# peterropac/Aegolius

Measured on AMD Instinct MI355X. Metric: Mpoints/sec SDF eval, 1024^3 grid, 10-prim smooth-union tree, higher is better.
Workload: dtype f32

## Files before the change

aegolius_amd/_engine.py:

```python
import atexit
import contextlib
import ctypes
import importlib.util
import os
import sys
import threading

import numpy as np

_HERE = os.path.dirname(os.path.abspath(__file__))
LIB_PATH = os.path.join(_HERE, "libsdfk.so")

MODE_AUTO, MODE_INTERPRET, MODE_SPECIALIZED, MODE_NOCULL = 0, 1, 2, 3
(FLAVOUR_PLAIN_ARRAY, FLAVOUR_PLAIN_GRID, FLAVOUR_TILE_ARRAY, FLAVOUR_TILE_GRID, FLAVOUR_TILE_MASK, FLAVOUR_ROWS_ARRAY,
 FLAVOUR_ROWS_GRID, FLAVOUR_ROWS_MASK, FLAVOUR_ROWS2D_ARRAY, FLAVOUR_ROWS2D_GRID, FLAVOUR_RAYS, FLAVOUR_OCCUPANCY) = range(12)
FLAVOUR_FLAGS = 0x100
FLAVOUR_XY = 0x200

_c = ctypes
_vp, _i64, _int, _sz = _c.c_void_p, _c.c_int64, _c.c_int, _c.c_size_t
_fp = _c.POINTER(_c.c_float)

SIGNATURES = {
    "sdfk_abi_version": (_int, []),
    "sdfk_device_count": (_int, []),
    "sdfk_last_error": (_c.c_char_p, []),
    "sdfk_program_create": (_vp, [_vp, _sz, _vp, _sz, _vp, _sz, _int]),
    "sdfk_program_destroy": (None, [_vp]),
    "sdfk_program_set_params": (_int, [_vp, _vp, _sz]),
    "sdfk_program_set_cull": (_int, [_vp, _vp, _sz, _vp]),
    "sdfk_program_source": (_c.c_char_p, [_vp]),
    "sdfk_program_compile_check": (_int, [_vp, _c.POINTER(_sz)]),
    "sdfk_program_chain_members": (_int, [_vp]),
    "sdfk_program_compile_flavour": (_int, [_vp, _int, _c.POINTER(_sz), _c.POINTER(_c.c_double)]),
    "sdfk_debug_compile_external": (_int, [_vp, _int, _c.POINTER(_sz)]),
    "sdfk_debug_jit_stats": (None, [_c.POINTER(_i64), _c.POINTER(_c.c_double)]),
    "sdfk_jit_drain": (None, []),
    "sdfk_jit_cancel": (None, []),
    "sdfk_debug_set_rtc_defs": (None, [_c.c_char_p]),
    "sdfk_eval_device": (_int, [_vp, _vp, _i64, _i64, _vp, _vp, _int]),
    "sdfk_eval_device_rows": (_int, [_vp, _vp, _i64, _i64, _i64, _vp, _vp, _int]),
    "sdfk_eval_device_rows2d": (_int, [_vp, _vp, _i64, _i64, _i64, _vp, _vp, _int]),
    "sdfk_eval_device_rows2d_xy": (_int, [_vp, _vp, _i64, _i64, _i64, _vp, _vp, _int]),
    "sdfk_debug_cells_stats": (None, [_int, _c.POINTER(_c.c_longlong)]),
    "sdfk_debug_rays_stats": (None, [_int, _c.POINTER(_c.c_longlong)]),
    "sdfk_eval_device_rows3d": (_int, [_vp, _vp, _i64, _i64, _i64, _i64, _i64, _vp, _vp, _int]),
    "sdfk_debug_row_masks": (_int, [_vp, _vp, _i64, _i64, _i64, _vp, _c.POINTER(_i64), _c.POINTER(_int), _vp]),
    "sdfk_eval_grid_sharded": (_int, [_vp, _vp, _i64, _vp, _i64, _vp, _i64, _int, _vp, _vp, _int]),
    "sdfk_eval_grid_sharded_device": (_int, [_vp, _vp, _i64, _vp, _i64, _vp, _i64, _int, _vp, _int, _vp, _int]),
    "sdfk_eval_device_aux": (_int, [_vp, _vp, _i64, _i64, _vp, _int, _i64, _vp, _vp, _int]),
    "sdfk_eval_grid_aux": (_int, [_vp, _vp, _i64, _vp, _i64, _vp, _i64, _i64, _i64, _vp, _int, _i64, _vp, _vp, _int]),
    "sdfk_field_min": (_int, [_vp, _i64, _c.POINTER(_c.c_float), _vp]),
    "sdfk_grid_box_average": (_int, [_vp, _i64, _i64, _i64, _int, _int, _int, _int, _vp, _vp]),
    "sdfk_grid_edge_detect": (_int, [_vp, _i64, _i64, _i64, _vp, _vp]),
    "sdfk_debug_box_variant": (_int, [_i64, _i64, _i64, _int, _int, _int, _c.POINTER(_int)]),
    "sdfk_grid_signed": (_int, [_vp, _i64, _i64, _i64, _c.c_float, _int, _vp, _vp]),
    "sdfk_grid_boundary_mask": (_int, [_vp, _i64, _c.c_float, _vp, _vp]),
    "sdfk_grid_signed_slab": (_int, [_vp, _i64, _i64, _vp, _i64, _i64, _i64, _int, _vp, _vp]),
    "sdfk_eval_host": (_int, [_vp, _vp, _int, _i64, _i64, _vp, _int, _int]),
# ... 141 lines not shown


def check(rc, what):
    if rc != 0:
        raise SdfkError("%s failed (%d): %s" % (what, rc, last_error()))


def device_count():
    return lib().sdfk_device_count()


def require_gpu():
    if device_count() < 1:
        raise SdfkError("aegolius_amd: no HIP device visible - SDF evaluation runs on an MI355X only "
                        "(there is no CPU path)")


def jit_stats():
    n, t = _i64(0), _c.c_double(0.0)
    lib().sdfk_debug_jit_stats(ctypes.byref(n), ctypes.byref(t))
    return n.value, t.value


def _ptr(a):
    return a.ctypes.data_as(_vp) if a is not None and a.size else None


def _release(owner, attr, destroy):
    try:
        h = getattr(owner, attr, None)
        setattr(owner, attr, None)
        if h and _lib is not None:
            getattr(_lib, destroy)(_vp(h))
    except Exception:
        pass


def coords_n(shape):
    if len(shape) != 2 or shape[0] != 3:
        raise ValueError("coordinates must have shape (3, N); got %r" % (tuple(shape),))
    return int(shape[1])


def host_coords(co, dtype=None):
    co = np.asarray(co)
    coords_n(co.shape)
# ... 543 lines not shown
```

aegolius_amd/csrc/sdfk.hip:

```cpp
#include <hip/hip_runtime.h>
#include <hip/hiprtc.h>

#include <chrono>
#include <algorithm>
#include <atomic>
#include <cmath>
#include <condition_variable>
#include <cstdio>
#include <cstdlib>
#include <cstring>
#include <deque>
#include <functional>
#include <map>
#include <memory>
#include <mutex>
#include <thread>
#include <string>
#include <vector>
#include <dirent.h>
#include <dlfcn.h>
#include <fcntl.h>
#include <signal.h>
#include <spawn.h>
#include <sys/wait.h>
// ... 989 lines not shown
        std::lock_guard<std::mutex> lk(mu);
        jobs.clear();
        cv.notify_all();
    }
    ~BuildWorker() {
        {
            std::lock_guard<std::mutex> lk(mu);
            stop = true;
            cv.notify_all();
        }
        for (std::thread& t : threads)
            if (t.joinable()) t.join();
    }
};
static BuildWorker g_builds;
extern "C" void sdfk_jit_drain(void) { g_builds.drain(); }
extern "C" void sdfk_jit_cancel(void) {
    g_cancel_builds.store(true);
    g_builds.drop_queued();
    g_builds.drain();
}
static std::atomic<long long> g_compile_count{0};
static std::atomic<long long> g_compile_micros{0};
extern "C" void sdfk_debug_jit_stats(int64_t* builds, double* seconds) {
    if (builds) *builds = g_compile_count.load();
    if (seconds) *seconds = (double)g_compile_micros.load() * 1e-6;
}

static std::shared_ptr<CodeObject> code_entry(const std::string& key) {
    std::lock_guard<std::mutex> lk(g_code_mu);
    std::shared_ptr<CodeObject>& e = g_code[key];
    if (!e) e = std::make_shared<CodeObject>();
    return e;
}
static void code_build(const std::shared_ptr<CodeObject>& e, const std::string& src, int rwb, bool external = false) {
    const auto t0 = std::chrono::steady_clock::now();
    std::vector<char> co;
    std::string log;
    bool from_disk = false;
    std::string disk_path;
    const int rc = rtc_compile(src, &co, &log, rwb, &from_disk, &disk_path, external);
    const double dt = std::chrono::duration<double>(std::chrono::steady_clock::now() - t0).count();
    if (!from_disk) {
        g_compile_count++;
        g_compile_micros += (long long)(dt * 1e6);
    }
// ... 10 lines not shown
    }
    e->cv.notify_all();
}
template <typename MakeSource>
static std::shared_ptr<CodeObject> code_get(const std::string& key, MakeSource make_source, int rwb, bool wait) {
    std::shared_ptr<CodeObject> e = code_entry(key);
    std::unique_lock<std::mutex> lk(e->mu);
    if (e->state == 3 && std::chrono::steady_clock::now() - e->failed_at > std::chrono::seconds(30)) e->state = 0;
    if (e->state == 0) {
        e->state = 1;
        lk.unlock();
        const std::string src = make_source();
        if (wait || !rtc_helper_available()) {
            code_build(e, src, rwb);
        } else {
            g_builds.post([e, src, rwb] { code_build(e, src, rwb, true); });
        }
        return e;
    }
    if (wait) e->cv.wait(lk, [&] { return e->state != 1; });
    return e;
}
static std::string flavour_key(const sdfk_program* p, int flavour, int rwb, int with_flags = 0) {
    return p->key + "|f" + std::to_string(flavour) + ((with_flags & 1) ? "s" : "") + ((with_flags & 2) ? "x" : "") + "|" + rtc_option_key(rwb);
}
static std::string flavour_source(const sdfk_program* p, int flavour, int with_flags = 0) {
    return std::string((with_flags & 1) ? "#define SDFK_FLAGS 1\n" : "") + ((with_flags & 2) ? "#define SDFK_XY 1\n" : "") +
           sdfk_generate_source(g_ops, SDFK_OP_COUNT, p->code.data(), p->code.size() / 2, p->result_reg, p->sites, flavour,
                                &p->sites_all);
}

extern "C" int sdfk_program_chain_members(const sdfk_program* p) {
    return p && p->chain_mode ? p->chain_members : 0;
}
extern "C" int sdfk_program_compile_check(sdfk_program* p, size_t* code_size) {
    if (!p) return fail(-1, "null program");
    size_t total = 0;
    const int rwb = rows_geo(p);
    for (int f = 0; f < SDFK_FL_COUNT; ++f) {
        if (f == SDFK_FL_RAYS) continue;
        if (f == SDFK_FL_OCCUPANCY) continue;
        if (p->sites.empty() && f != SDFK_FL_PLAIN_ARRAY && f != SDFK_FL_PLAIN_GRID) continue;
        if (p->chain_mode && (f == SDFK_FL_TILE_ARRAY || f == SDFK_FL_TILE_GRID || f == SDFK_FL_TILE_MASK || f == SDFK_FL_ROWS_MASK)) continue;
        std::shared_ptr<CodeObject> e = code_get(flavour_key(p, f, rwb), [&] { return flavour_source(p, f); }, rwb, true);
        if (e->state != 2) return fail(-3, e->error);
        total += e->co.size();
    }
    if (code_size) *code_size = total;
    return 0;
}
extern "C" int sdfk_program_compile_flavour(sdfk_program* p, int flavour, size_t* code_size, double* seconds) {
    if (!p) return fail(-1, "null program");
    int with_flags = 0;
    if (flavour >= 0 && (flavour & SDFK_FLAVOUR_FLAGS)) with_flags |= 1;
    if (flavour >= 0 && (flavour & SDFK_FLAVOUR_XY)) with_flags |= 2;
    if (flavour >= 0) flavour &= ~(SDFK_FLAVOUR_FLAGS | SDFK_FLAVOUR_XY);
    if (flavour < 0 || flavour >= SDFK_FL_COUNT) return fail(-1, "sdfk_program_compile_flavour: unknown flavour");
    if (p->sites.empty() && flavour != SDFK_FL_PLAIN_ARRAY && flavour != SDFK_FL_PLAIN_GRID && flavour != SDFK_FL_RAYS &&
        flavour != SDFK_FL_OCCUPANCY)
        return fail(-2, "sdfk_program_compile_flavour: the program has no cull sites");
    if (with_flags && flavour == SDFK_FL_RAYS)
        return fail(-2, "sdfk_program_compile_flavour: the ray flavour has no flag-writing or two-row build");
    if (with_flags && flavour == SDFK_FL_OCCUPANCY)
        return fail(-2, "sdfk_program_compile_flavour: the occupancy flavour has no flag-writing or two-row build");
    if ((with_flags & 2) && flavour != SDFK_FL_PLAIN_ARRAY && flavour != SDFK_FL_ROWS2D_ARRAY)
        return fail(-2, "sdfk_program_compile_flavour: two-row coordinates exist for the plain and the flat row-block array kernels");
    if ((with_flags & 1) && (flavour == SDFK_FL_TILE_ARRAY || flavour == SDFK_FL_TILE_GRID || flavour == SDFK_FL_TILE_MASK ||
                       flavour == SDFK_FL_ROWS_MASK))
        return fail(-2, "sdfk_program_compile_flavour: this flavour has no flag-writing build");
    const int rwb = rows_geo(p);
    const auto t0 = std::chrono::steady_clock::now();
    std::shared_ptr<CodeObject> e =
        code_get(flavour_key(p, flavour, rwb, with_flags), [&] { return flavour_source(p, flavour, with_flags); }, rwb, true);
    if (e->state != 2) return fail(-3, e->error);
    if (code_size) *code_size = e->co.size();
    if (seconds) *seconds = std::chrono::duration<double>(std::chrono::steady_clock::now() - t0).count();
    return 0;
}

extern "C" int sdfk_debug_compile_external(sdfk_program* p, int flavour, size_t* code_size) {
    if (!p) return fail(-1, "null program");
    if (flavour < 0 || flavour >= SDFK_FL_COUNT) return fail(-1, "sdfk_debug_compile_external: unknown flavour");
    if (p->sites.empty() && flavour != SDFK_FL_PLAIN_ARRAY && flavour != SDFK_FL_PLAIN_GRID && flavour != SDFK_FL_RAYS &&
// ... 261 lines not shown
        for (const uint2& x : sp) {
            if (x.y == 0xffffffffu) ++all;
            else { sum += x.y; mx = std::max<unsigned long long>(mx, x.y); if (x.y == 0) ++empty; }
        }
        {
            std::lock_guard<std::mutex> lk(g_cells_stats_mu);
            g_cells_stats[0] = (long long)nf; g_cells_stats[1] = (long long)nc; g_cells_stats[2] = (long long)head;
            g_cells_stats[3] = (long long)cap; g_cells_stats[4] = (long long)sum; g_cells_stats[5] = (long long)mx;
            g_cells_stats[6] = (long long)all; g_cells_stats[7] = (long long)empty;
        }
        if (trace) fprintf(stderr, "[sdfk cells] %d members: fine %ux%ux%u = %llu cells (2^%u planes x 2^%u blocks x 2^%u windows), coarse %llu; pool %u of %llu entries; "
                "fine lists: mean %.1f max %llu, %llu without a list, %llu empty\n", p->chain_members, fine.ncx, fine.ncy, fine.ncz, nf, fine.lx, fine.ly, fine.lz, nc,
                head, cap, (double)sum / (double)std::max<unsigned long long>(1, nf - all - empty), mx, all, empty);
    }
    out->lv = fine;
    out->sph = b + o_fsph;
    out->span = b + o_fspan;
    out->cand = b + o_pool;
    out->enabled = 1u;
    out->ncells = (unsigned)nf;
    return 0;
}

static int run(sdfk_program* p, const SrcArray* arr, const SrcGrid* grid, long long n, float* d_out, void* stream_,
               int mode, bool vec_ok, long long row_len = 0, const float* aux = nullptr, long long aux_stride = 0,
               bool flat = false, long long plane_rows = 0, long long plane_phase = 0, unsigned* d_flags = nullptr,
               unsigned thr_key = 0, bool xy = false) {
    if (!p) return fail(-1, "null program");
    if (n < 0) return fail(-1, "negative point count");
    if (p->n_aux > 0 && (!aux || aux_stride < n))
        return fail(-1, "this program reads auxiliary fields (staged evaluation): use sdfk_eval_device_aux / sdfk_eval_grid_aux");
    if (n == 0) return 0;
    if (mode == SDFK_MODE_AUTO) mode = g_default_mode;
    if (d_flags && (mode == SDFK_MODE_AUTO || mode == SDFK_MODE_INTERPRET)) mode = SDFK_MODE_SPECIALIZED;
    if (xy) {
        if (!arr || p->n_aux > 0) return fail(-1, "two-row coordinates: array source, no auxiliary fields");
        if (mode == SDFK_MODE_AUTO || mode == SDFK_MODE_INTERPRET) mode = SDFK_MODE_SPECIALIZED;
    }
    hipStream_t stream = (hipStream_t)stream_;
    int device = 0;
    HIPCHK(hipGetDevice(&device));
    DevState* d = nullptr;
    int rc = ensure_resident(p, device, stream, &d);
    if (rc) return rc;

    long long n4 = vec_ok ? (n / 4) * 4 : 0;
    long long tail = n - n4;

    static const long long spec_limit = [] {
        const char* e = getenv("SDFK_SPECIALIZE_LIMIT");
// ... 7 lines not shown
    }();
    if (mode == SDFK_MODE_AUTO && (long long)(p->code.size() / 2) > spec_limit && p->interp_ok && !p->chain_mode && !d_flags)
        mode = SDFK_MODE_INTERPRET;

    RowGeom rg;
    int flavour = arr ? SDFK_FL_PLAIN_ARRAY : SDFK_FL_PLAIN_GRID;
    const long long grow = grid ? (grid->n2 > 1 ? (long long)grid->n2 : (long long)grid->n1) : 0;
    if (!p->sites.empty() && mode != SDFK_MODE_NOCULL && mode != SDFK_MODE_INTERPRET) {
        if (arr && rows_geometry(n, row_len, &rg, (flat || d_flags) ? 0 : plane_rows, plane_phase, p->chain_mode))
            flavour = (flat || xy) ? SDFK_FL_ROWS2D_ARRAY : SDFK_FL_ROWS_ARRAY;
        else if (arr && vec_ok && !p->chain_mode && !d_flags && !xy) flavour = SDFK_FL_TILE_ARRAY;
        else if (grid && grid->start % grow == 0 &&
                 rows_geometry(n, grow, &rg, (grid->n2 > 1 && !d_flags) ? (long long)grid->n1 : 0,
                               grid->n2 > 1 ? (grid->start / grow) % (long long)grid->n1 : 0, p->chain_mode))
            flavour = grid->n2 > 1 ? SDFK_FL_ROWS_GRID : SDFK_FL_ROWS2D_GRID;
        else if (grid && vec_ok && !p->chain_mode && !d_flags) flavour = SDFK_FL_TILE_GRID;
        if (!p->chain_mode && (long long)(p->code.size() / 2) > rows_limit &&
            (flavour == SDFK_FL_ROWS_ARRAY || flavour == SDFK_FL_ROWS2D_ARRAY || flavour == SDFK_FL_ROWS_GRID || flavour == SDFK_FL_ROWS2D_GRID)) {
            const bool is_arr = arr != nullptr;
            if (vec_ok && !d_flags && !xy) flavour = is_arr ? SDFK_FL_TILE_ARRAY : SDFK_FL_TILE_GRID;
            else if (!d_flags) flavour = is_arr ? SDFK_FL_PLAIN_ARRAY : SDFK_FL_PLAIN_GRID;
        }
    }
    std::shared_ptr<SpecModule> sk;
    if (mode != SDFK_MODE_INTERPRET) {
        static const bool async_jit = [] { const char* e = getenv("SDFK_ASYNC_JIT"); return !(e && e[0] == '0'); }();
        const bool wait = mode != SDFK_MODE_AUTO || !p->interp_ok || !async_jit;
        std::string err;
        sk = get_module(p, device, flavour, wait, &err, (d_flags ? 1 : 0) | (xy ? 2 : 0));
        if (sk && sk->failed) {
            if (mode == SDFK_MODE_SPECIALIZED || !p->interp_ok)
                return fail(-3, "specialised kernel unavailable: " + err);
            static bool warned = false;
            if (!warned) {
                fprintf(stderr, "[sdfk] hiprtc specialisation failed, using the interpreter kernel: %s\n", err.c_str());
                warned = true;
            }
            sk.reset();
        }
    }
    if (!sk && !p->interp_ok)
        return fail(-4, "program needs more registers than the interpreter kernel has (use the specialised mode)");

    const float* prm = d->d_params;
    const float* tab = d->d_tables;
    if (sk) {
        if (flavour == SDFK_FL_ROWS_ARRAY || flavour == SDFK_FL_ROWS_GRID || flavour == SDFK_FL_ROWS2D_ARRAY ||
            flavour == SDFK_FL_ROWS2D_GRID) {
            const unsigned per_tile = (unsigned)(rows_waves(p) * rows_wbricks(p));
            const unsigned tiles = ((rg.nbricks + per_tile - 1) / per_tile + 127u) & ~127u;
            const unsigned rthreads = 64u * (unsigned)rows_waves(p);
            CellsArg cells{};
            const bool with_cells = p->chain_mode && sk->fn[1] != nullptr;
            if (arr) {
                const float* co = arr->co;
                long long stride = arr->stride;
                if (with_cells) {
                    void* src[] = {&co, &stride};
                    rc = prepare_cells(p, d, sk->fn[1], rg, src, 2, prm, tab, stream, &cells);
                    if (rc) return rc;
                }
                void* args[] = {&prm, &tab, &co, &stride, &rg, &d_out, &d_flags, &thr_key, &cells};
                HIPCHK(hipModuleLaunchKernel(sk->fn[0], tiles, 1, 1, rthreads, 1, 1, 0, stream, args, nullptr));
            } else {
                SrcGrid g = *grid;
                rg.row0 = grid->start / grow;
                rg.yrows = grid->n2 > 1 ? 0 : 1;
                if (with_cells) {
                    void* src[] = {&g};
                    rc = prepare_cells(p, d, sk->fn[1], rg, src, 1, prm, tab, stream, &cells);
                    if (rc) return rc;
                }
                void* args[] = {&prm, &tab, &g, &rg, &d_out, &d_flags, &thr_key, &cells};
                HIPCHK(hipModuleLaunchKernel(sk->fn[0], tiles, 1, 1, rthreads, 1, 1, 0, stream, args, nullptr));
            }
            return 0;
        }
        if (flavour == SDFK_FL_TILE_ARRAY || flavour == SDFK_FL_TILE_GRID) {
            const unsigned tiles = (unsigned)((n + tile_points() - 1) / tile_points());
            if (arr) {
                const float* co = arr->co;
                long long stride = arr->stride;
                void* args[] = {&prm, &tab, &co, &stride, &n, &d_out};
                HIPCHK(hipModuleLaunchKernel(sk->fn[0], tiles, 1, 1, tile_threads(), 1, 1, 0, stream, args, nullptr));
            } else {
                SrcGrid g = *grid;
                void* args[] = {&prm, &tab, &g, &n, &d_out};
                HIPCHK(hipModuleLaunchKernel(sk->fn[0], tiles, 1, 1, tile_threads(), 1, 1, 0, stream, args, nullptr));
            }
            return 0;
        }
        if (arr) {
            const float* co = arr->co;
            long long stride = arr->stride;
            if (n4) {
                long long off = 0;
                void* args[] = {&prm, &tab, &co, &stride, &off, &n4, &d_out, &aux, &aux_stride, &d_flags, &thr_key};
// ... 173 lines not shown
    return 0;
}

extern "C" int sdfk_linspace_f32(double lo, double hi, int64_t n, float* out) {
    if (n < 0 || (n > 0 && !out)) return fail(-1, "sdfk_linspace_f32: bad arguments");
    if (n == 0) return 0;
    if (n == 1) {
        out[0] = (float)lo;
        return 0;
    }
    const double div = (double)(n - 1);
    const double delta = hi - lo;
    const double step = delta / div;
    for (int64_t i = 0; i < n; ++i) {
        volatile double t = (step != 0.0) ? (double)i * step : ((double)i / div) * delta;
        out[i] = (float)(t + lo);
    }
    out[n - 1] = (float)hi;
    return 0;
}

struct AxisTables {
    float* d = nullptr;
    ~AxisTables() {
        if (d) (void)hipFree(d);
    }
};

static int upload_axes(const float* ax0, int64_t n0, const float* ax1, int64_t n1, const float* ax2, int64_t n2,
                       hipStream_t stream, AxisTables* t, SrcGrid* g, int64_t start) {
    if (!ax0 || !ax1 || !ax2 || n0 < 1 || n1 < 1 || n2 < 1) return fail(-1, "grid axes missing or empty");
    if (n1 > 0x7fffffff || n2 > 0x7fffffff) return fail(-1, "grid axis too long");
    HIPCHK(hipMalloc(&t->d, (size_t)(n0 + n1 + n2) * sizeof(float)));
    HIPCHK(hipMemcpyAsync(t->d, ax0, (size_t)n0 * sizeof(float), hipMemcpyHostToDevice, stream));
    HIPCHK(hipMemcpyAsync(t->d + n0, ax1, (size_t)n1 * sizeof(float), hipMemcpyHostToDevice, stream));
    HIPCHK(hipMemcpyAsync(t->d + n0 + n1, ax2, (size_t)n2 * sizeof(float), hipMemcpyHostToDevice, stream));
    g->ax0 = t->d;
    g->ax1 = t->d + n0;
    g->ax2 = t->d + n0 + n1;
    g->n1 = (unsigned)n1;
    g->n2 = (unsigned)n2;
    g->start = start;
    return 0;
}

extern "C" int sdfk_eval_grid(sdfk_program* p, const float* ax0, int64_t n0, const float* ax1, int64_t n1,
                              const float* ax2, int64_t n2, int64_t start, int64_t count, float* d_out, void* stream,
                              int mode) {
    if (!d_out) return fail(-1, "sdfk_eval_grid: null output");
    if (start < 0 || count < 0 || start + count > n0 * n1 * n2) return fail(-1, "sdfk_eval_grid: range outside the grid");
    AxisTables t;
    SrcGrid g;
    int rc = upload_axes(ax0, n0, ax1, n1, ax2, n2, (hipStream_t)stream, &t, &g, start);
    if (rc) return rc;
    rc = run(p, nullptr, &g, count, d_out, stream, mode, aligned16(d_out));
    if (rc) return rc;
    HIPCHK(hipStreamSynchronize((hipStream_t)stream));
    return 0;
}

extern "C" int sdfk_eval_grid_aux(sdfk_program* p, const float* ax0, int64_t n0, const float* ax1, int64_t n1,
                                  const float* ax2, int64_t n2, int64_t start, int64_t count, const float* d_aux, int n_aux,
                                  int64_t aux_stride, float* d_out, void* stream, int mode) {
    if (!p || !d_out) return fail(-1, "sdfk_eval_grid_aux: null pointer");
    if (start < 0 || count < 0 || start + count > n0 * n1 * n2) return fail(-1, "sdfk_eval_grid_aux: range outside the grid");
    if (n_aux < p->n_aux) return fail(-1, "sdfk_eval_grid_aux: the program reads more auxiliary fields than were passed");
    AxisTables t;
    SrcGrid g;
    int rc = upload_axes(ax0, n0, ax1, n1, ax2, n2, (hipStream_t)stream, &t, &g, start);
    if (rc) return rc;
    rc = run(p, nullptr, &g, count, d_out, stream, mode, aligned16(d_out), 0, d_aux, aux_stride);
    if (rc) return rc;
    HIPCHK(hipStreamSynchronize((hipStream_t)stream));
    return 0;
}

extern "C" int sdfk_eval_grid_host(sdfk_program* p, const float* ax0, int64_t n0, const float* ax1, int64_t n1,
                                   const float* ax2, int64_t n2, int64_t start, int64_t count, float* out, int device,
                                   int mode) {
    if (!p) return fail(-1, "null program");
    if (count < 0 || (count > 0 && !out)) return fail(-1, "sdfk_eval_grid_host: bad arguments");
    if (start < 0 || start + count > n0 * n1 * n2) return fail(-1, "sdfk_eval_grid_host: range outside the grid");
    if (count == 0) return 0;
    HIPCHK(hipSetDevice(device));
    int64_t chunk = std::min<int64_t>(count, (int64_t)1 << 27);
    const int64_t grow = n2 > 1 ? n2 : n1;
    if (start % grow == 0 && chunk > grow) chunk = chunk / grow * grow;
    float* d_out = nullptr;
    HIPCHK(hipMalloc(&d_out, (size_t)chunk * sizeof(float)));
    AxisTables t;
    SrcGrid g;
    int rc = upload_axes(ax0, n0, ax1, n1, ax2, n2, nullptr, &t, &g, start);
    for (int64_t s = 0; s < count && rc == 0; s += chunk) {
        const int64_t m = std::min(chunk, count - s);
        g.start = start + s;
        rc = run(p, nullptr, &g, m, d_out, nullptr, mode, true);
        if (rc == 0 && hipMemcpy(out + s, d_out, (size_t)m * sizeof(float), hipMemcpyDeviceToHost) != hipSuccess)
            rc = fail(-6, "sdfk_eval_grid_host: device-to-host copy failed");
    }
    (void)hipFree(d_out);
    return rc;
}

extern "C" int sdfk_eval_grid_sharded(sdfk_program* p, const float* ax0, int64_t n0, const float* ax1, int64_t n1,
                                      const float* ax2, int64_t n2, int n_shards, const int* devices, float* out,
                                      int mode) {
    if (!p || !out) return fail(-1, "sdfk_eval_grid_sharded: null argument");
    if (n_shards < 1 || n_shards > 64) return fail(-1, "sdfk_eval_grid_sharded: 1..64 shards");
    if (!ax0 || !ax1 || !ax2 || n0 < 1 || n1 < 1 || n2 < 1) return fail(-1, "grid axes missing or empty");
    int n_dev = 0;
    if (hipGetDeviceCount(&n_dev) != hipSuccess || n_dev < 1) return fail(-8, "sdfk_eval_grid_sharded: no HIP device");
    const int64_t total = n0 * n1 * n2, unit = n2 > 1 ? n2 : n1;
    const int64_t per = (total / unit / n_shards) * unit;
    std::vector<int> rc((size_t)n_shards, 0);
    std::vector<std::string> msg((size_t)n_shards);
    std::vector<std::thread> workers;
    for (int d = 0; d < n_shards; ++d) {
        const int dev = devices ? devices[d] : d % n_dev;
        if (dev < 0 || dev >= n_dev) return fail(-1, "sdfk_eval_grid_sharded: device index out of range");
// ... 361 lines not shown
```

aegolius_amd/csrc/sdfk_codegen.cpp:

```cpp
#include "sdfk_codegen.h"

#include <algorithm>
#include <cstdio>
#include <cstring>
#include <map>
#include <set>

#include "sdfk_embedded.inc"

std::string sdfk_vector_prelude() { return std::string(kEmbeddedDevice) + "\n" + kEmbeddedVecdev + "\n"; }

static const char kWrappers[] = R"SDFKW(
template <int VEC, typename SRC>
static __device__ __forceinline__ void sdfk_body(const float* __restrict__ PRM, const float* __restrict__ TAB,
                                                 const SRC& src, long long off, long long n,
                                                 float* __restrict__ out, const float* __restrict__ aux,
                                                 long long aux_stride, unsigned* __restrict__ flags, unsigned thr) {
    const long long block_base = (long long)sdfk_bx() * (SDFK_BLOCK * VEC);
    const unsigned lane_off = sdfk_tx() * VEC;
#ifdef SDFK_FLAGS                                              // the flag-writing build of this flavour (its own code object:
    {                                                          // carried as a run-time branch it cost the field kernels registers)
        const bool active = block_base + lane_off < n;
        unsigned nib = 0u;
        if (active) {
// ... 903 lines not shown
            d2s = sd_rawmax(d2s, sd_rawmax(sd_rawmax(ea.x, ea.y), sd_rawmax(eb.x, eb.y)));
#endif
        }
    }
    const float r2 = sdfk_wave_max(d2);
#ifdef SDFK_CELLS
    // inside: max |p - S| <= radius of S, with room for the rounding of the distances (relative 1e-5; S.w < 0: no cell)
    const float rs2 = sdfk_wave_max(d2s);
    if (lane == 0) meta->inside[b] = (S.w > 0.0f && 1.00002f * sqrtf(rs2) <= S.w) ? 1u : 0u;
#endif
    if (lane == 0) {
#ifdef SDFK_FLAT
        meta->bound[b] = make_float4(cx, cz, cy, 1.00001f * sqrtf(r2) + 1e-30f);
#else
        meta->bound[b] = make_float4(cx, cy, cz, 1.00001f * sqrtf(r2) + 1e-30f);
#endif
        meta->uniform[b] = uniform ? 1u : 0u;
#ifdef SDFK_SIMT
#pragma unroll
        for (int w = 0; w < SDFK_NMASK; ++w) meta->mask[w][b] = ~0ull;   // the fold lanes AND their decisions into these
#endif
    }
}
#if defined(SDFK_SIMT) && SDFK_NSUB > 1
// Probe centre `sb` of brick b whose rows each have one x and one y: the sub-brick is rows [r0, r0 + RPS) x points
// [i0, i0 + ZPS) of the window; sphere around the midpoint of its first and last point, radius = the exact maximum
// over its points (read back from the staged coordinates), so any input is bounded correctly — on a regular grid
// 4 rows x 8 points have a quarter of the brick's radius.
static __device__ __forceinline__ float4 sdfk_sub_centre(const sdfk_rowmeta* meta, unsigned b, unsigned sb) {
    constexpr int NZP = 4, NRP = SDFK_NSUB / NZP, RPS = SDFK_RROWS / NRP, ZPS = SDFK_RZ / NZP;
    static_assert(ZPS % 4 == 0 && RPS >= 1, "sub-brick shape");
    int r0 = (int)(sb / NZP) * RPS, r1 = r0 + RPS;
    const int i0 = (int)(sb % NZP) * ZPS;
    if constexpr (NRP == 2) {
        // A brick whose 16 rows come from TWO planes of the grid (1 row block in 32 at 513^3: the last rows of one plane,
        // y near its maximum, and the first rows of the next, y near its minimum) is split where x changes instead of in the
        // middle: each part lies in one plane and is bounded tightly; split in the middle, the part that holds the plane
        // change spans the whole y extent and nothing of the brick could be culled.
        const float x0 = meta->xy[b][0].x;
        if (__builtin_bit_cast(unsigned, x0) != __builtin_bit_cast(unsigned, meta->xy[b][SDFK_RROWS - 1].x)) {
            int s = 1;
            while (s < SDFK_RROWS - 1 && __builtin_bit_cast(unsigned, meta->xy[b][s].x) == __builtin_bit_cast(unsigned, x0)) ++s;
            r0 = sb / NZP ? s : 0;
            r1 = sb / NZP ? SDFK_RROWS : s;
        }
    }
// ... 140 lines not shown
        meta->nalive[b] = n_out <= SDFK_ALIST_CAP ? n_out : (listed ? SDFK_LIST_ALIVE : SDFK_ALL_ALIVE);
        meta->aspan[b] = make_uint2(off, cnt);
    }
}
#endif

// phases A and B of the tile of this workgroup; returns this wave's first brick (row block, window)
#ifdef SDFK_CELLS
#define SDFK_CELLS_PARAM , const sdfk_cells& cl
#define SDFK_CELLS_PASS , cl
#else
#define SDFK_CELLS_PARAM
#define SDFK_CELLS_PASS
#endif
template <typename SRC>
static __device__ __forceinline__ void sdfk_rows_prepare(const float* __restrict__ PRM, const float* __restrict__ TAB,
                                                         const SRC& s, const sdfk_rowgeom& g, sdfk_rowmeta* meta,
                                                         unsigned tile, unsigned& rb0, unsigned& c0 SDFK_CELLS_PARAM) {
    const int lane = sdfk_tx() & 63, wave = __builtin_amdgcn_readfirstlane(sdfk_tx() >> 6);
    const unsigned q0 = tile * SDFK_RNBRICK + wave * SDFK_RWBRICKS;            // first brick of this wave
    rb0 = sdfk_udiv(q0, g.nchunk, g.inv_nchunk);                // (back in an SGPR: what is derived from it stays scalar)
    c0 = q0 - rb0 * g.nchunk;
    unsigned rb = rb0, c = c0;
#if SDFK_RWBRICKS <= 2 && !defined(SDFK_NOHOIST)
    // two-wave workgroups on the north-star grid; with four bricks per wave the registers this takes cost more)
    sdfk_rowregs hregs[SDFK_RWBRICKS];
    bool live[SDFK_RWBRICKS];
#ifdef SDFK_CELLS
    uint2 cspan[SDFK_RWBRICKS];
    unsigned cfirst[SDFK_RWBRICKS];
    float4 csph[SDFK_RWBRICKS];
#endif
#pragma unroll
    for (int j = 0; j < SDFK_RWBRICKS; ++j) {
        long long r0, rend;
#ifdef SDFK_CELLS
        sdfk_brick_cell(g, cl, rb, c, r0, rend, cspan[j], csph[j]);
        cfirst[j] = 0u;                                          // the lane's entry of the list's first batch: in flight with the coordinates
        if (cspan[j].y != SDFK_ALL_ALIVE && (unsigned)lane < cspan[j].y) cfirst[j] = cl.cand[cspan[j].x + (unsigned)lane];
#else
        sdfk_block_rows(g, rb, r0, rend);
#endif
        live[j] = q0 + j < g.nbricks && r0 < rend;               // (blocks of the last plane beyond the slab: nothing)
        if (live[j]) sdfk_rows_load(s, g, r0, rend, c, lane, hregs[j]);
        if (++c == g.nchunk) { c = 0; ++rb; }
    }
#pragma unroll
// ... 145 lines not shown
    const unsigned xg_t = sdfk_bx() / 8;
    const unsigned tile = (((xg_t / SDFK_XGROUP) * 8 + sdfk_bx() % 8) * SDFK_XGROUP + xg_t % SDFK_XGROUP) * SDFK_RTILES + tt;
    if (tile * SDFK_RNBRICK >= g.nbricks) break;
    if (tt) __syncthreads();
    unsigned rb, c;
    sdfk_rows_prepare(PRM, TAB, s, g, &meta, tile, rb, c SDFK_CELLS_PASS);
    const unsigned q0 = tile * SDFK_RNBRICK + wave * SDFK_RWBRICKS;
#pragma unroll 1
    for (int j = 0; j < SDFK_RWBRICKS; ++j) {
        if (q0 + j >= g.nbricks) break;
        const int b = wave * SDFK_RWBRICKS + j;
        const unsigned k = c;
        long long r0, rend;
        sdfk_block_rows(g, rb, r0, rend);
        if (++c == g.nchunk) { c = 0; ++rb; }
        if (r0 >= rend) continue;
        unsigned mw[2 * SDFK_NMASK];                             // the brick's skip bits as scalar words
#pragma unroll
        for (int w = 0; w < SDFK_NMASK; ++w) {
            const unsigned long long m = meta.mask[w][b];
            mw[2 * w] = __builtin_amdgcn_readfirstlane((unsigned)m);
            mw[2 * w + 1] = __builtin_amdgcn_readfirstlane((unsigned)(m >> 32));
        }
        const bool uniform = __builtin_amdgcn_readfirstlane(meta.uniform[b]) != 0u;
        const bool interior = sdfk_interior(g.L, k);
#ifdef SDFK_ABLATE_EDGE
        if (!interior) continue;
#endif
        const bool live_row = r0 + lr < rend;
        const int dr = live_row ? lr : (int)(rend - 1 - r0);
        long long f;                                              // flat index of this lane's first point
        const int z = sdfk_win_z(r0 + dr, g.L, k, zq, &f);        // its index in the row (edge chunks: may lie outside)
        const int last = (int)g.L - 1;
        V3P P[SDFK_NP];
        f2 res[SDFK_NP];
        // the staged coordinate: z (SDFK_FLAT: y, see sdfk_rows_load)
#ifdef SDFK_FLAT
        SDFK_EACH P[q].y = *reinterpret_cast<const f2*>(&meta.z[b][lr * SDFK_RZ + zq + 2 * q]);
#else
        SDFK_EACH P[q].z = *reinterpret_cast<const f2*>(&meta.z[b][lr * SDFK_RZ + zq + 2 * q]);
#endif
#ifdef SDFK_ABLATE_EVAL
        if (true) {
#ifdef SDFK_FLAT
            SDFK_EACH res[q] = P[q].y + __builtin_bit_cast(float, mw[0] ^ mw[1] ^ mw[2] ^ mw[3]);
#else
            SDFK_EACH res[q] = P[q].z + __builtin_bit_cast(float, mw[0] ^ mw[1] ^ mw[2] ^ mw[3]);
#endif
        } else
#endif
        if (uniform) {
            const float2 xy = meta.xy[b][lr];
#ifdef SDFK_FLAT
            SDFK_EACH { P[q].x = sp<f2>(xy.x); P[q].z = sp<f2>(xy.y); }      // (x, 0)
#else
            SDFK_EACH { P[q].x = sp<f2>(xy.x); P[q].y = sp<f2>(xy.y); }
#endif
#ifndef SDFK_CHAIN
            sdfk_rows_culled<true>(xy.x, xy.y, P, mw, PRM, TAB, res);
#endif
        } else {                                                  // the other coordinates of every point again (L2-resident)
#pragma unroll
            for (int q = 0; q < SDFK_NP; q += 2) {
                float4 X, Y, Z;
                sdfk_rows_fetch(s, g, r0, dr, z + 2 * q, interior, X, Y, Z);
                P[q].x = {X.x, X.y};
                P[q + 1].x = {X.z, X.w};
#ifdef SDFK_FLAT
                P[q].z = {Z.x, Z.y};
                P[q + 1].z = {Z.z, Z.w};
#else
                P[q].y = {Y.x, Y.y};
                P[q + 1].y = {Y.z, Y.w};
#endif
            }
#ifndef SDFK_CHAIN
            sdfk_rows_culled<false>(0.0f, 0.0f, P, mw, PRM, TAB, res);
#endif
        }
#ifdef SDFK_CHAIN
        {   // The children on the brick's list, in order; the first one starts the accumulator. Looked up one by one — kind of
            // the child, base of its parameters, then the parameters: three dependent scalar loads per child — the evaluation
            // the next SDFK_CHUNK children lane-parallel — a lane per (child, parameter) — into LDS, and then evaluates them
            // from there: the latency is paid once per chunk.
#ifdef SDFK_CELLS
            // (more survivors than the list holds — nalive = ALL —: every member, in order, straight from its index)
            const unsigned nal = __builtin_amdgcn_readfirstlane(meta.nalive[b]);
            const bool all_alive = nal == SDFK_ALL_ALIVE, list_alive = nal == SDFK_LIST_ALIVE;
            const unsigned aoff = __builtin_amdgcn_readfirstlane(meta.aspan[b].x);
            const unsigned cnt = all_alive ? (unsigned)SDFK_NLEAF : (list_alive ? __builtin_amdgcn_readfirstlane(meta.aspan[b].y) : nal);
#define SDFK_AREC(i) (all_alive ? sdfk_member_record(i) : (list_alive ? cl.cand[aoff + (i)] : meta.alist[b][i]))
#else
            const unsigned cnt = __builtin_amdgcn_readfirstlane(meta.nalive[b]);
#define SDFK_AREC(i) sdfk_member_record((unsigned)meta.alist[b][i])
#endif
            f2 acc[SDFK_NP];
#if SDFK_CHAIN_STAGED
            if (cnt <= SDFK_STAGE_MIN)
#endif
            {
                // one or two survivors (the 50-child flat union: 1.06 per brick): staging costs more than it hides, and
                // parameters in SGPRs beat parameters read back from LDS — straight from the table
// ... 1326 lines not shown
```

include/sdfk.h:

```cpp
#ifndef SDFK_H
#define SDFK_H

#include <stddef.h>
#include <stdint.h>

#ifdef __cplusplus
extern "C" {
#endif

#define SDFK_ABI_VERSION 1

#define SDFK_MODE_AUTO 0
#define SDFK_MODE_INTERPRET 1
#define SDFK_MODE_SPECIALIZED 2
#define SDFK_MODE_NOCULL 3

typedef struct sdfk_program sdfk_program;

int sdfk_abi_version(void);
int sdfk_device_count(void);
const char* sdfk_last_error(void);

sdfk_program* sdfk_program_create(const uint32_t* code, size_t n_instr, const float* params, size_t n_params,
                                  const float* tables, size_t n_tables, int result_reg);
void sdfk_program_destroy(sdfk_program* prog);
int sdfk_program_set_params(sdfk_program* prog, const float* params, size_t n_params);
int sdfk_program_set_cull(sdfk_program* prog, const uint32_t* sites, size_t n_sites, const float* k);
int sdfk_program_chain_members(const sdfk_program* prog);
const char* sdfk_program_source(sdfk_program* prog);
int sdfk_program_compile_check(sdfk_program* prog, size_t* code_size);
#define SDFK_FLAVOUR_PLAIN_ARRAY 0
#define SDFK_FLAVOUR_PLAIN_GRID 1
#define SDFK_FLAVOUR_TILE_ARRAY 2
#define SDFK_FLAVOUR_TILE_GRID 3
#define SDFK_FLAVOUR_TILE_MASK 4
#define SDFK_FLAVOUR_ROWS_ARRAY 5
#define SDFK_FLAVOUR_ROWS_GRID 6
#define SDFK_FLAVOUR_ROWS_MASK 7
#define SDFK_FLAVOUR_ROWS2D_ARRAY 8
#define SDFK_FLAVOUR_ROWS2D_GRID 9
#define SDFK_FLAVOUR_RAYS 10
#define SDFK_FLAVOUR_OCCUPANCY 11
#define SDFK_FLAVOUR_FLAGS 0x100
#define SDFK_FLAVOUR_XY 0x200
int sdfk_program_compile_flavour(sdfk_program* prog, int flavour, size_t* code_size, double* seconds);
void sdfk_debug_cells_stats(int enable, long long* out8);
void sdfk_debug_rays_stats(int enable, long long* out8);
int sdfk_debug_compile_external(sdfk_program* prog, int flavour, size_t* code_size);
void sdfk_jit_drain(void);
void sdfk_jit_cancel(void);
void sdfk_debug_jit_stats(int64_t* builds, double* seconds);
void sdfk_debug_set_rtc_defs(const char* defs);

int sdfk_eval_device(sdfk_program* prog, const float* d_co, int64_t n, int64_t row_stride, float* d_out,
                     void* stream, int mode);
int sdfk_eval_device_rows(sdfk_program* prog, const float* d_co, int64_t n, int64_t row_stride, int64_t row_len,
                          float* d_out, void* stream, int mode);
int sdfk_eval_device_rows3d(sdfk_program* prog, const float* d_co, int64_t n, int64_t row_stride, int64_t row_len,
                            int64_t plane_rows, int64_t first_row_in_plane, float* d_out, void* stream, int mode);
int sdfk_eval_device_rows2d(sdfk_program* prog, const float* d_co, int64_t n, int64_t row_stride, int64_t row_len,
                            float* d_out, void* stream, int mode);
int sdfk_eval_device_rows2d_xy(sdfk_program* prog, const float* d_xy, int64_t n, int64_t row_stride, int64_t row_len,
                               float* d_out, void* stream, int mode);
int sdfk_eval_host(sdfk_program* prog, const void* co, int co_dtype, int64_t n, int64_t row_stride, float* out,
                   int device, int mode);
int sdfk_eval_host_resident(sdfk_program* prog, const void* co, int co_dtype, int64_t n, int64_t row_stride,
                            float* d_out, int device, int mode);
int sdfk_eval_grid(sdfk_program* prog, const float* ax0, int64_t n0, const float* ax1, int64_t n1, const float* ax2,
                   int64_t n2, int64_t start, int64_t count, float* d_out, void* stream, int mode);
int sdfk_eval_grid_host(sdfk_program* prog, const float* ax0, int64_t n0, const float* ax1, int64_t n1,
                        const float* ax2, int64_t n2, int64_t start, int64_t count, float* out, int device, int mode);
int sdfk_eval_grid_sharded(sdfk_program* prog, const float* ax0, int64_t n0, const float* ax1, int64_t n1,
                           const float* ax2, int64_t n2, int n_shards, const int* devices, float* out, int mode);
int sdfk_eval_grid_sharded_device(sdfk_program* prog, const float* ax0, int64_t n0, const float* ax1, int64_t n1,
// ... 170 lines not shown
```

Before: 367,100.

## Add lattice build of row-grid kernel exploiting per-row uniform x/y on axis grids

```diff
diff --git a/aegolius_amd/_engine.py b/aegolius_amd/_engine.py
--- a/aegolius_amd/_engine.py
+++ b/aegolius_amd/_engine.py
@@ -16,6 +16,7 @@
  FLAVOUR_ROWS_GRID, FLAVOUR_ROWS_MASK, FLAVOUR_ROWS2D_ARRAY, FLAVOUR_ROWS2D_GRID, FLAVOUR_RAYS, FLAVOUR_OCCUPANCY) = range(12)
 FLAVOUR_FLAGS = 0x100
 FLAVOUR_XY = 0x200
+FLAVOUR_LATTICE = 0x400
 
 _c = ctypes
 _vp, _i64, _int, _sz = _c.c_void_p, _c.c_int64, _c.c_int, _c.c_size_t
@@ -35,6 +36,7 @@
     "sdfk_program_compile_flavour": (_int, [_vp, _int, _c.POINTER(_sz), _c.POINTER(_c.c_double)]),
     "sdfk_debug_compile_external": (_int, [_vp, _int, _c.POINTER(_sz)]),
     "sdfk_debug_jit_stats": (None, [_c.POINTER(_i64), _c.POINTER(_c.c_double)]),
+    "sdfk_debug_lattice_stats": (None, [_c.POINTER(_i64)]),
     "sdfk_jit_drain": (None, []),
     "sdfk_jit_cancel": (None, []),
     "sdfk_debug_set_rtc_defs": (None, [_c.c_char_p]),
@@ -222,6 +224,12 @@
     return n.value, t.value
 
 
+def lattice_stats():
+    n = _i64(0)
+    lib().sdfk_debug_lattice_stats(ctypes.byref(n))
+    return n.value
+
+
 def _ptr(a):
     return a.ctypes.data_as(_vp) if a is not None and a.size else None
 
diff --git a/aegolius_amd/csrc/sdfk.hip b/aegolius_amd/csrc/sdfk.hip
--- a/aegolius_amd/csrc/sdfk.hip
+++ b/aegolius_amd/csrc/sdfk.hip
@@ -1035,6 +1035,10 @@
 }
 static std::atomic<long long> g_compile_count{0};
 static std::atomic<long long> g_compile_micros{0};
+static std::atomic<long long> g_lattice_launches{0};
+extern "C" void sdfk_debug_lattice_stats(int64_t* launches) {
+    if (launches) *launches = g_lattice_launches.load();
+}
 extern "C" void sdfk_debug_jit_stats(int64_t* builds, double* seconds) {
     if (builds) *builds = g_compile_count.load();
     if (seconds) *seconds = (double)g_compile_micros.load() * 1e-6;
@@ -1091,10 +1095,12 @@
     return e;
 }
 static std::string flavour_key(const sdfk_program* p, int flavour, int rwb, int with_flags = 0) {
-    return p->key + "|f" + std::to_string(flavour) + ((with_flags & 1) ? "s" : "") + ((with_flags & 2) ? "x" : "") + "|" + rtc_option_key(rwb);
+    return p->key + "|f" + std::to_string(flavour) + ((with_flags & 1) ? "s" : "") + ((with_flags & 2) ? "x" : "") + ((with_flags & 4) ? "l" : "") + "|" +
+           rtc_option_key(rwb);
 }
 static std::string flavour_source(const sdfk_program* p, int flavour, int with_flags = 0) {
     return std::string((with_flags & 1) ? "#define SDFK_FLAGS 1\n" : "") + ((with_flags & 2) ? "#define SDFK_XY 1\n" : "") +
+           ((with_flags & 4) ? "#define SDFK_LATTICE 1\n" : "") +
            sdfk_generate_source(g_ops, SDFK_OP_COUNT, p->code.data(), p->code.size() / 2, p->result_reg, p->sites, flavour,
                                 &p->sites_all);
 }
@@ -1123,11 +1129,15 @@
     int with_flags = 0;
     if (flavour >= 0 && (flavour & SDFK_FLAVOUR_FLAGS)) with_flags |= 1;
     if (flavour >= 0 && (flavour & SDFK_FLAVOUR_XY)) with_flags |= 2;
-    if (flavour >= 0) flavour &= ~(SDFK_FLAVOUR_FLAGS | SDFK_FLAVOUR_XY);
+    if (flavour >= 0 && (flavour & SDFK_FLAVOUR_LATTICE)) with_flags |= 4;
+    if (flavour >= 0) flavour &= ~(SDFK_FLAVOUR_FLAGS | SDFK_FLAVOUR_XY | SDFK_FLAVOUR_LATTICE);
     if (flavour < 0 || flavour >= SDFK_FL_COUNT) return fail(-1, "sdfk_program_compile_flavour: unknown flavour");
     if (p->sites.empty() && flavour != SDFK_FL_PLAIN_ARRAY && flavour != SDFK_FL_PLAIN_GRID && flavour != SDFK_FL_RAYS &&
         flavour != SDFK_FL_OCCUPANCY)
         return fail(-2, "sdfk_program_compile_flavour: the program has no cull sites");
+    if ((with_flags & 4) && (flavour != SDFK_FL_ROWS_GRID || with_flags != 4 || p->chain_mode))
+        return fail(-2, "sdfk_program_compile_flavour: the lattice build exists for the field-writing 3-D axis-table row-block "
+                        "kernel of programs that are not chains");
     if (with_flags && flavour == SDFK_FL_RAYS)
         return fail(-2, "sdfk_program_compile_flavour: the ray flavour has no flag-writing or two-row build");
     if (with_flags && flavour == SDFK_FL_OCCUPANCY)
@@ -1435,10 +1445,14 @@
     return 0;
 }
 
+static bool lattice_off() {
+    const char* e = getenv("SDFK_NO_LATTICE");
+    return e && e[0] == '1';
+}
 static int run(sdfk_program* p, const SrcArray* arr, const SrcGrid* grid, long long n, float* d_out, void* stream_,
                int mode, bool vec_ok, long long row_len = 0, const float* aux = nullptr, long long aux_stride = 0,
                bool flat = false, long long plane_rows = 0, long long plane_phase = 0, unsigned* d_flags = nullptr,
-               unsigned thr_key = 0, bool xy = false) {
+               unsigned thr_key = 0, bool xy = false, bool grid_monotone = false) {
     if (!p) return fail(-1, "null program");
     if (n < 0) return fail(-1, "negative point count");
     if (p->n_aux > 0 && (!aux || aux_stride < n))
@@ -1492,12 +1506,14 @@
             else if (!d_flags) flavour = is_arr ? SDFK_FL_PLAIN_ARRAY : SDFK_FL_PLAIN_GRID;
         }
     }
+    const bool lattice = flavour == SDFK_FL_ROWS_GRID && grid && grid->n2 > 1 && grid_monotone && !p->chain_mode && !d_flags &&
+                         !aux && p->n_aux == 0 && !lattice_off();
     std::shared_ptr<SpecModule> sk;
     if (mode != SDFK_MODE_INTERPRET) {
         static const bool async_jit = [] { const char* e = getenv("SDFK_ASYNC_JIT"); return !(e && e[0] == '0'); }();
         const bool wait = mode != SDFK_MODE_AUTO || !p->interp_ok || !async_jit;
         std::string err;
-        sk = get_module(p, device, flavour, wait, &err, (d_flags ? 1 : 0) | (xy ? 2 : 0));
+        sk = get_module(p, device, flavour, wait, &err, (d_flags ? 1 : 0) | (xy ? 2 : 0) | (lattice ? 4 : 0));
         if (sk && sk->failed) {
             if (mode == SDFK_MODE_SPECIALIZED || !p->interp_ok)
                 return fail(-3, "specialised kernel unavailable: " + err);
@@ -1543,6 +1559,7 @@
                 }
                 void* args[] = {&prm, &tab, &g, &rg, &d_out, &d_flags, &thr_key, &cells};
                 HIPCHK(hipModuleLaunchKernel(sk->fn[0], tiles, 1, 1, rthreads, 1, 1, 0, stream, args, nullptr));
+                if (lattice) g_lattice_launches.fetch_add(1);
             }
             return 0;
         }
@@ -1762,11 +1779,20 @@
 
 struct AxisTables {
     float* d = nullptr;
+    bool monotone = false;
     ~AxisTables() {
         if (d) (void)hipFree(d);
     }
 };
 
+static bool axis_monotone(const float* a, int64_t n) {
+    bool up = true, down = true;
+    for (int64_t i = 1; i < n; ++i) {
+        up = up && a[i - 1] <= a[i];
+        down = down && a[i - 1] >= a[i];
+    }
+    return up || down;
+}
 static int upload_axes(const float* ax0, int64_t n0, const float* ax1, int64_t n1, const float* ax2, int64_t n2,
                        hipStream_t stream, AxisTables* t, SrcGrid* g, int64_t start) {
     if (!ax0 || !ax1 || !ax2 || n0 < 1 || n1 < 1 || n2 < 1) return fail(-1, "grid axes missing or empty");
@@ -1775,6 +1801,7 @@
     HIPCHK(hipMemcpyAsync(t->d, ax0, (size_t)n0 * sizeof(float), hipMemcpyHostToDevice, stream));
     HIPCHK(hipMemcpyAsync(t->d + n0, ax1, (size_t)n1 * sizeof(float), hipMemcpyHostToDevice, stream));
     HIPCHK(hipMemcpyAsync(t->d + n0 + n1, ax2, (size_t)n2 * sizeof(float), hipMemcpyHostToDevice, stream));
+    t->monotone = axis_monotone(ax0, n0) && axis_monotone(ax1, n1) && axis_monotone(ax2, n2);
     g->ax0 = t->d;
     g->ax1 = t->d + n0;
     g->ax2 = t->d + n0 + n1;
@@ -1793,7 +1820,7 @@
     SrcGrid g;
     int rc = upload_axes(ax0, n0, ax1, n1, ax2, n2, (hipStream_t)stream, &t, &g, start);
     if (rc) return rc;
-    rc = run(p, nullptr, &g, count, d_out, stream, mode, aligned16(d_out));
+    rc = run(p, nullptr, &g, count, d_out, stream, mode, aligned16(d_out), 0, nullptr, 0, false, 0, 0, nullptr, 0, false, t.monotone);
     if (rc) return rc;
     HIPCHK(hipStreamSynchronize((hipStream_t)stream));
     return 0;
@@ -1834,7 +1861,7 @@
     for (int64_t s = 0; s < count && rc == 0; s += chunk) {
         const int64_t m = std::min(chunk, count - s);
         g.start = start + s;
-        rc = run(p, nullptr, &g, m, d_out, nullptr, mode, true);
+        rc = run(p, nullptr, &g, m, d_out, nullptr, mode, true, 0, nullptr, 0, false, 0, 0, nullptr, 0, false, t.monotone);
         if (rc == 0 && hipMemcpy(out + s, d_out, (size_t)m * sizeof(float), hipMemcpyDeviceToHost) != hipSuccess)
             rc = fail(-6, "sdfk_eval_grid_host: device-to-host copy failed");
     }
diff --git a/aegolius_amd/csrc/sdfk_codegen.cpp b/aegolius_amd/csrc/sdfk_codegen.cpp
--- a/aegolius_amd/csrc/sdfk_codegen.cpp
+++ b/aegolius_amd/csrc/sdfk_codegen.cpp
@@ -949,6 +949,133 @@
 #endif
     }
 }
+#ifdef SDFK_LATTICE
+// ---- the lattice build of sdfk_spec_rg (3-D axis-table grids; field out, no chain) ----------------------------------------
+// On a grid that is expanded from three tables every row has one x and one y BY CONSTRUCTION, so phase A neither builds
+// x / y quads nor tests them: (ix, iy) of the brick's first row come from one wave-uniform division per row block, the 16
+// row-head lanes fetch the rows' x and y for meta.xy, and all of a wave's table reads are issued before the first is used.
+// The LDS layout, the probe and phase C are those of the array-era build; phase C loses its non-uniform half.
+#if defined(SDFK_FLAT) || defined(SDFK_CHAIN) || defined(SDFK_FLAGS) || defined(SDFK_XY)
+#error "SDFK_LATTICE: only the field-writing, non-chain build of the 3-D axis-table row-block kernel"
+#endif
+#if defined(SDFK_SIMT) && SDFK_NSUB > 1
+#define SDFK_LAT_HEADS 1                          // the probe bounds sub-bricks from LDS: only the row heads need x and y
+#else
+#define SDFK_LAT_HEADS 0                          // one sphere around the whole brick: every lane needs its row's x and y
+#endif
+struct sdfk_latregs {
+    float4 Z[SDFK_RLOADS];
+    int z[SDFK_RLOADS];                           // index in its row of the quad's first point (edge windows: may lie outside)
+    float x[SDFK_RLOADS], y[SDFK_RLOADS];         // of the lane's row (SDFK_LAT_HEADS: valid in the row-head lanes only)
+};
+// (ix, iy) of global row g.row0 + r0, wave-uniform, back in SGPRs. Row counts beyond 2^32 take the 64-bit division.
+static __device__ __forceinline__ void sdfk_lat_divmod(const SrcGrid& s, const sdfk_rowgeom& g, long long r0,
+                                                       unsigned long long& ix, unsigned& iy0) {
+    const unsigned long long g0 = (unsigned long long)(g.row0 + r0);
+    if ((g0 >> 32) == 0ull) {
+        const unsigned q = (unsigned)g0 / s.n1;
+        ix = __builtin_amdgcn_readfirstlane(q);
+        iy0 = __builtin_amdgcn_readfirstlane((unsigned)g0 - q * s.n1);
+    } else {
+        const unsigned long long q = g0 / s.n1;
+        ix = ((unsigned long long)__builtin_amdgcn_readfirstlane((unsigned)(q >> 32)) << 32) |
+             (unsigned long long)__builtin_amdgcn_readfirstlane((unsigned)q);
+        iy0 = __builtin_amdgcn_readfirstlane((unsigned)(g0 - q * s.n1));
+    }
+}
+// phase A, part 1: the table reads of one brick (rows [r0, rend) of one row block, window k; ix, iy0: of row r0)
+static __device__ __forceinline__ void sdfk_lat_load(const SrcGrid& s, const sdfk_rowgeom& g, long long r0, long long rend,
+                                                     unsigned k, unsigned long long ix, unsigned iy0, int lane, sdfk_latregs& r) {
+    const bool interior = sdfk_interior(g.L, k);
+    const int last = (int)g.L - 1;
+    const int nr = rend - r0 < (long long)SDFK_RROWS ? (int)(rend - r0) : SDFK_RROWS;     // rows of this block (>= 1)
+    const unsigned rlo = (unsigned)r0;                         // (row * L) mod 32 needs the low bits of the row only
+#pragma unroll
+    for (int t = 0; t < SDFK_RLOADS; ++t) {
+        int dr = 8 * t + (lane >> 3);
+        if (dr >= nr) dr = nr - 1;
+        // the window's first point in this row (sdfk_win_z): 32 k - (row * L) mod 32, plus the lane's 4 points
+        const int z = (int)(32u * k) + 4 * (lane & 7) - (int)(((rlo + (unsigned)dr) * g.L) & 31u);
+        // ONE 16-byte read per quad in every window, no branch around it: the quad [zc, zc + 4) nearest to [z, z + 4) inside
+        // the row (L >= 32) holds every element that the clamped reads of an edge window would fetch (sdfk_lat_edge)
+        const int zc = interior ? z : min(max(z, 0), last - 3);
+        const sdfk_f4u v = *reinterpret_cast<const sdfk_f4u*>(s.ax2 + zc);
+        r.Z[t] = make_float4(v.x, v.y, v.z, v.w);
+        r.z[t] = z;
+        r.x[t] = 0.0f;
+        r.y[t] = 0.0f;
+        if (!SDFK_LAT_HEADS || (lane & 7) == 0) {
+            unsigned long long jx = ix;
+            unsigned iy = iy0 + (unsigned)dr;
+            while (iy >= s.n1) { iy -= s.n1; ++jx; }           // (blocks that span planes: n1 < 16, no plane hint)
+            r.x[t] = s.ax0[jx];
+            r.y[t] = s.ax1[iy];
+        }
+    }
+}
+// edge windows: element e of the quad is the row's point clamp(z + e, 0, last) — the duplicates of the array build — picked
+// from the quad that was read at zc = clamp(z, 0, last - 3)
+static __device__ __forceinline__ float sdfk_lat_pick(const float4& q, int d) {
+    // d in 0 .. 3. Bit masks (three v_bfi), not ?: — the compiler turns a chain of selects on d into a jump table or an
+    // array in scratch memory
+    const unsigned m1 = (unsigned)((int)((unsigned)d << 31) >> 31), m2 = (unsigned)((int)((unsigned)d << 30) >> 31);
+    const unsigned x = __builtin_bit_cast(unsigned, q.x), y = __builtin_bit_cast(unsigned, q.y);
+    const unsigned z = __builtin_bit_cast(unsigned, q.z), w = __builtin_bit_cast(unsigned, q.w);
+    const unsigned lo = (y & m1) | (x & ~m1), hi = (w & m1) | (z & ~m1);
+    return __builtin_bit_cast(float, (hi & m2) | (lo & ~m2));
+}
+static __device__ __forceinline__ void sdfk_lat_edge(sdfk_latregs& r, int last) {
+#pragma unroll
+    for (int t = 0; t < SDFK_RLOADS; ++t) {
+        const int z = r.z[t], zc = min(max(z, 0), last - 3);
+        const float4 q = r.Z[t];
+        r.Z[t] = make_float4(sdfk_lat_pick(q, min(max(z, 0), last) - zc), sdfk_lat_pick(q, min(max(z + 1, 0), last) - zc),
+                             sdfk_lat_pick(q, min(max(z + 2, 0), last) - zc), sdfk_lat_pick(q, min(max(z + 3, 0), last) - zc));
+    }
+}
+// phase A, part 2: z and the row heads to LDS as the array build leaves them; the sphere around the whole brick where
+// the probe still asks for it (same centre, same radius, same margins as sdfk_rows_bounds on a uniform brick)
+static __device__ __forceinline__ void sdfk_lat_bounds(const sdfk_latregs& r, int lane, sdfk_rowmeta* meta, int b) {
+#pragma unroll
+    for (int t = 0; t < SDFK_RLOADS; ++t) {
+        *reinterpret_cast<float4*>(&meta->z[b][(8 * t + (lane >> 3)) * SDFK_RZ + 4 * (lane & 7)]) = r.Z[t];
+        if ((lane & 7) == 0) meta->xy[b][8 * t + (lane >> 3)] = make_float2(r.x[t], r.y[t]);
+    }
+#ifdef SDFK_ABLATE_BOUNDS
+    if (lane == 0) { meta->bound[b] = make_float4(0.f, 0.f, 0.f, 1.f); meta->uniform[b] = 1u; }
+    return;
+#endif
+#if SDFK_LAT_HEADS
+    if (lane == 0) {
+        meta->uniform[b] = 1u;
+#pragma unroll
+        for (int w = 0; w < SDFK_NMASK; ++w) meta->mask[w][b] = ~0ull;
+    }
+#else
+    const float cx = 0.5f * (sdfk_lane(r.x[0], 0) + sdfk_lane(r.x[SDFK_RLOADS - 1], 63));
+    const float cy = 0.5f * (sdfk_lane(r.y[0], 0) + sdfk_lane(r.y[SDFK_RLOADS - 1], 63));
+    const float cz = 0.5f * (sdfk_lane(r.Z[0].x, 0) + sdfk_lane(r.Z[SDFK_RLOADS - 1].w, 63));
+    float d2 = 0.0f;
+#pragma unroll
+    for (int t = 0; t < SDFK_RLOADS; ++t) {                     // |p - c|^2 = dxy^2 + max |z - cz|^2
+        const float dx = r.x[t] - cx, dy = r.y[t] - cy;
+        const float zm = sd_rawmax(sd_rawmax(sd_abs(r.Z[t].x - cz), sd_abs(r.Z[t].y - cz)),
+                                   sd_rawmax(sd_abs(r.Z[t].z - cz), sd_abs(r.Z[t].w - cz)));
+        d2 = sd_rawmax(d2, sd_fma(zm, zm, sd_fma(dx, dx, dy * dy)));
+    }
+    const float r2 = sdfk_wave_max(d2);
+    if (lane == 0) {
+        meta->bound[b] = make_float4(cx, cy, cz, 1.00001f * sqrtf(r2) + 1e-30f);
+        meta->uniform[b] = 1u;
+#ifdef SDFK_SIMT
+#pragma unroll
+        for (int w = 0; w < SDFK_NMASK; ++w) meta->mask[w][b] = ~0ull;
+#endif
+    }
+#endif
+}
+#endif
+
 #if defined(SDFK_SIMT) && SDFK_NSUB > 1
 // Probe centre `sb` of brick b whose rows each have one x and one y: the sub-brick is rows [r0, r0 + RPS) x points
 // [i0, i0 + ZPS) of the window; sphere around the midpoint of its first and last point, radius = the exact maximum
@@ -1135,7 +1262,34 @@
     rb0 = sdfk_udiv(q0, g.nchunk, g.inv_nchunk);                // (back in an SGPR: what is derived from it stays scalar)
     c0 = q0 - rb0 * g.nchunk;
     unsigned rb = rb0, c = c0;
-#if SDFK_RWBRICKS <= 2 && !defined(SDFK_NOHOIST)
+#ifdef SDFK_LATTICE
+    // every table read of the wave's bricks is in flight before the first one is used; the division comes first and is
+    // shared by the bricks of one row block
+    sdfk_latregs lregs[SDFK_RWBRICKS];
+    bool live[SDFK_RWBRICKS], edge[SDFK_RWBRICKS];
+    unsigned long long lat_ix = 0ull;
+    unsigned lat_iy0 = 0u;
+    bool lat_have = false;
+#pragma unroll
+    for (int j = 0; j < SDFK_RWBRICKS; ++j) {
+        long long r0, rend;
+        sdfk_block_rows(g, rb, r0, rend);
+        live[j] = q0 + j < g.nbricks && r0 < rend;
+        edge[j] = !sdfk_interior(g.L, c);
+        if (live[j]) {
+            if (!lat_have || c == 0u) sdfk_lat_divmod(s, g, r0, lat_ix, lat_iy0);   // (c == 0: the first brick of a new row block)
+            lat_have = true;
+            sdfk_lat_load(s, g, r0, rend, c, lat_ix, lat_iy0, lane, lregs[j]);
+        }
+        if (++c == g.nchunk) { c = 0; ++rb; }
+    }
+#pragma unroll
+    for (int j = 0; j < SDFK_RWBRICKS; ++j)
+        if (live[j]) {
+            if (edge[j]) sdfk_lat_edge(lregs[j], (int)g.L - 1);
+            sdfk_lat_bounds(lregs[j], lane, meta, wave * SDFK_RWBRICKS + j);
+        } else if (lane == 0) { meta->bound[wave * SDFK_RWBRICKS + j] = make_float4(0.0f, 0.0f, 0.0f, 1.0f); meta->uniform[wave * SDFK_RWBRICKS + j] = 0u; }   // (masks: never read)
+#elif SDFK_RWBRICKS <= 2 && !defined(SDFK_NOHOIST)
     // two-wave workgroups on the north-star grid; with four bricks per wave the registers this takes cost more)
     sdfk_rowregs hregs[SDFK_RWBRICKS];
     bool live[SDFK_RWBRICKS];
@@ -1327,7 +1481,11 @@
             mw[2 * w] = __builtin_amdgcn_readfirstlane((unsigned)m);
             mw[2 * w + 1] = __builtin_amdgcn_readfirstlane((unsigned)(m >> 32));
         }
+#ifdef SDFK_LATTICE
+        constexpr bool uniform = true;                            // by construction: the other half of phase C is not built
+#else
         const bool uniform = __builtin_amdgcn_readfirstlane(meta.uniform[b]) != 0u;
+#endif
         const bool interior = sdfk_interior(g.L, k);
 #ifdef SDFK_ABLATE_EDGE
         if (!interior) continue;
@@ -1364,7 +1522,9 @@
 #ifndef SDFK_CHAIN
             sdfk_rows_culled<true>(xy.x, xy.y, P, mw, PRM, TAB, res);
 #endif
-        } else {                                                  // the other coordinates of every point again (L2-resident)
+        }
+#ifndef SDFK_LATTICE
+        else {                                                    // the other coordinates of every point again (L2-resident)
 #pragma unroll
             for (int q = 0; q < SDFK_NP; q += 2) {
                 float4 X, Y, Z;
@@ -1383,6 +1543,7 @@
             sdfk_rows_culled<false>(0.0f, 0.0f, P, mw, PRM, TAB, res);
 #endif
         }
+#endif
 #ifdef SDFK_CHAIN
         {   // The children on the brick's list, in order; the first one starts the accumulator. Looked up one by one — kind of
             // the child, base of its parameters, then the parameters: three dependent scalar loads per child — the evaluation
diff --git a/include/sdfk.h b/include/sdfk.h
--- a/include/sdfk.h
+++ b/include/sdfk.h
@@ -43,6 +43,7 @@
 #define SDFK_FLAVOUR_OCCUPANCY 11
 #define SDFK_FLAVOUR_FLAGS 0x100
 #define SDFK_FLAVOUR_XY 0x200
+#define SDFK_FLAVOUR_LATTICE 0x400
 int sdfk_program_compile_flavour(sdfk_program* prog, int flavour, size_t* code_size, double* seconds);
 void sdfk_debug_cells_stats(int enable, long long* out8);
 void sdfk_debug_rays_stats(int enable, long long* out8);
@@ -50,6 +51,7 @@
 void sdfk_jit_drain(void);
 void sdfk_jit_cancel(void);
 void sdfk_debug_jit_stats(int64_t* builds, double* seconds);
+void sdfk_debug_lattice_stats(int64_t* launches);
 void sdfk_debug_set_rtc_defs(const char* defs);
 
 int sdfk_eval_device(sdfk_program* prog, const float* d_co, int64_t n, int64_t row_stride, float* d_out,
```

Measured after the change: 367,100 (median of 4 runs). No clear change (-0.0%).
